# NinV/Background-Debiased-Video-CIL

Measured on AMD Instinct MI355X. Metric: clips/sec fwd+bwd TSM-R50 8x224^2 bs32/GPU, higher is better.
Workload: dtype f32; 1 GPU; TSM-ResNet50 fwd+bwd+SGD step, synthetic 32x8x3x224x224 clips per GPU, 101 classes, SimpleLinear+CrossEntropyLoss, dropout 0.5, random-init weights; fp32 tensors, accumulators and results; conv products: fp32 via 3xbf16 split, 6 MFMA products, fp32 accumulate (dropped terms <= 2^-24 relative); conv_arith=bf16x3, clips_per_gpu=32, global_batch=32, parallelism=dp1

## Files before the change

### background-debiased-video-cil_amd/csrc/conv_mfma.hip

```cpp
#include <stdlib.h>
#include "common.h"

#ifdef BDV_STAMPS
__device__ unsigned long long* g_stamp_buf = nullptr;
__device__ int g_stamp_cap = 0;
#define BDV_STAMP(slot)                                                                                                          \
  do {                                                                                                                           \
    if (threadIdx.x == 0 && g_stamp_buf != nullptr && (int)(blockIdx.x + gridDim.x * blockIdx.y) < g_stamp_cap) {                 \
      unsigned long long* q_ = g_stamp_buf + (size_t)(blockIdx.x + gridDim.x * blockIdx.y) * 8;                                  \
      if ((slot) == 4) asm volatile("s_waitcnt vmcnt(0)" ::: "memory");                                                          \
      q_[slot] = __builtin_amdgcn_s_memtime();                                                                                   \
      if ((slot) == 0) { q_[5] = __builtin_amdgcn_s_memrealtime(); q_[7] = __builtin_amdgcn_s_getreg((4 << 0) | (0 << 6) | (31 << 11)); } \
      if ((slot) == 4) q_[6] = __builtin_amdgcn_s_memrealtime();                                                                 \
    }                                                                                                                            \
  } while (0)
#else
#define BDV_STAMP(slot) do { } while (0)
#endif

namespace {

constexpr int BK = 32;

struct Geom {
  int N, H, W, Cin, Ho, Wo, Cout, R, S, stride, pad, pad_w, T, fold;
  int Rt, st_t;
  float rcp_RS, rcp_S;
  int M;
  int Ktot;
  float rcp_HoWo, rcp_Wo;
  int stagger;
};

typedef unsigned int u32x4 __attribute__((ext_vector_type(4)));
constexpr int kOOB = (int)0x80000000;

__device__ __forceinline__ float4 buf_load16(__amdgpu_buffer_rsrc_t rsrc, int voff, int soff) {
  const u32x4 v = __builtin_amdgcn_raw_buffer_load_b128(rsrc, voff, soff, 0);
  return make_float4(__uint_as_float(v.x), __uint_as_float(v.y), __uint_as_float(v.z), __uint_as_float(v.w));
}

__device__ __forceinline__ void buf_store16(__amdgpu_buffer_rsrc_t rsrc, int voff, float4 v) {
  u32x4 d;
  d.x = __float_as_uint(v.x);
  d.y = __float_as_uint(v.y);
  d.z = __float_as_uint(v.z);
  d.w = __float_as_uint(v.w);
  __builtin_amdgcn_raw_buffer_store_b128(d, rsrc, voff, 0, 0);
}

typedef unsigned int u32x2v __attribute__((ext_vector_type(2)));
template <int ES>
__device__ __forceinline__ float4 buf_ld4(__amdgpu_buffer_rsrc_t rsrc, int voff) {
  if constexpr (ES == 4) {
    return buf_load16(rsrc, voff, 0);
  } else {
    const u32x2v v = __builtin_amdgcn_raw_buffer_load_b64(rsrc, voff, 0, 0);
    return bdv_widen_bf16x4(v.x, v.y);
  }
}
template <int ES>
__device__ __forceinline__ void buf_st4(__amdgpu_buffer_rsrc_t rsrc, int voff, float4 v) {
  if constexpr (ES == 4) {
    buf_store16(rsrc, voff, v);
  } else {
    __builtin_amdgcn_raw_buffer_store_b64((u32x2v){bdv_pack_bf16x2(v.x, v.y), bdv_pack_bf16x2(v.z, v.w)}, rsrc, voff, 0, 0);
  }
}

__device__ __forceinline__ void fast_divmod(int m, int d, float rcp, int& q, int& r) {
  q = (int)((float)m * rcp);
  r = m - q * d;
  if (r < 0) {
    r += d;
    --q;
  }
  if (r >= d) {
    r -= d;
    ++q;
  }
}

template <int LDA, int LDB, int TM, int TN, int MS, int NS, bool SWA, bool SWB>
__device__ __forceinline__ void mma_stage(const float* __restrict__ As, const float* __restrict__ Bs,
                                          f32x16 (&acc)[TM][TN], int wm0, int wn0, int lane) {
  const int r = lane & 31, h = lane >> 5;
  const float* apv[SWA ? 8 : 1];
  const float* bpv[SWB ? 8 : 1];
#pragma unroll
  for (int c = 0; c < (SWA ? 8 : 1); ++c) apv[c] = As + h * LDA + wm0 + (r ^ (4 * c));
#pragma unroll
  for (int c = 0; c < (SWB ? 8 : 1); ++c) bpv[c] = Bs + h * LDB + wn0 + (r ^ (4 * c));
  auto ap = [&](int s, int i) { return apv[SWA ? ((s >> 1) & 7) : 0][2 * s * LDA + MS * i]; };
  auto bp = [&](int s, int j) { return bpv[SWB ? ((s >> 1) & 7) : 0][2 * s * LDB + NS * j]; };
  float a[2][TM], b[2][TN];
#pragma unroll
  for (int i = 0; i < TM; ++i) a[0][i] = ap(0, i);
#pragma unroll
  for (int j = 0; j < TN; ++j) b[0][j] = bp(0, j);
#pragma unroll
  for (int s = 0; s < BK / 2; ++s) {
    const int cur = s & 1, nxt = cur ^ 1;
    if (s + 1 < BK / 2) {
#pragma unroll
      for (int i = 0; i < TM; ++i) a[nxt][i] = ap(s + 1, i);
#pragma unroll
      for (int j = 0; j < TN; ++j) b[nxt][j] = bp(s + 1, j);
    }
#pragma unroll
    for (int i = 0; i < TM; ++i)
#pragma unroll
      for (int j = 0; j < TN; ++j)
        acc[i][j] = __builtin_amdgcn_mfma_f32_32x32x2f32(a[cur][i], b[cur][j], acc[i][j], 0, 0, 0);
    __builtin_amdgcn_sched_group_barrier(0x100, TM + TN, 0);
    __builtin_amdgcn_sched_group_barrier(0x008, TM * TN, 0);
  }
}

__device__ __forceinline__ int shift_class(int c, int fold) {
  return (fold > 0) ? (c < fold ? 1 : (c < 2 * fold ? -1 : 0)) : 0;
}

template <int LD, int PASSES>
__device__ __forceinline__ void store_transposed(float* __restrict__ dst, const float4 (&v)[PASSES], int tid) {
  const int row = tid >> 3, kg = tid & 7;
#pragma unroll
  for (int p = 0; p < PASSES; ++p) {
    float* d = dst + (4 * kg) * LD + ((row + 32 * p) ^ (4 * kg));
    d[0] = v[p].x;
    d[LD] = v[p].y;
    d[2 * LD] = v[p].z;
    d[3 * LD] = v[p].w;
  }
}

template <int LD, int COLS, int PASSES>
__device__ __forceinline__ void store_direct(float* __restrict__ dst, const float4 (&v)[PASSES], int tid) {
  constexpr int V = COLS / 4;
#pragma unroll
  for (int p = 0; p < PASSES; ++p) {
    const int idx = tid + 256 * p;
    const int krow = idx / V, c4 = idx - krow * V;
    *reinterpret_cast<float4*>(dst + krow * LD + 4 * c4) = v[p];
  }
}

__device__ __forceinline__ int acc_row(int reg, int lane) { return (reg & 3) + 8 * (reg >> 2) + 4 * (lane >> 5); }

struct Work {
  int dp_tiles, rem_tiles, split;
};

__device__ __forceinline__ int xcd_remap(int b, int n) {
  const int q = n >> 3, r = n & 7, x = b & 7, j = b >> 3;
  return (x < r ? x * (q + 1) : r * (q + 1) + (x - r) * q) + j;
}

struct WorkItem {
  int tile, kb, ke, pslot;
};

__device__ __forceinline__ WorkItem get_work(int b, const Work& wk, int nk) {
  WorkItem it;
  if (b < wk.dp_tiles) {
    it.tile = xcd_remap(b, wk.dp_tiles);
    it.kb = 0;
    it.ke = nk;
    it.pslot = -1;
  } else {
    const int rem = b - wk.dp_tiles;
    const int rt = rem / wk.split, sl = rem - rt * wk.split;
    it.tile = wk.dp_tiles + rt;
    it.kb = (int)(((long long)sl * nk) / wk.split);
    it.ke = (int)(((long long)(sl + 1) * nk) / wk.split);
    it.pslot = wk.split > 1 ? rem : -1;
  }
  return it;
}

template <int TM, int TN, int NT = 256>
__device__ __forceinline__ void store_partial(float* __restrict__ slab, int pslot, const f32x16 (&acc)[TM][TN], int tid) {
  float* base = slab + (size_t)pslot * (TM * TN * 16) * NT + tid;
#pragma unroll
  for (int i = 0; i < TM; ++i)
#pragma unroll
    for (int j = 0; j < TN; ++j)
#pragma unroll
      for (int e = 0; e < 16; ++e) base[(size_t)((i * TN + j) * 16 + e) * NT] = acc[i][j][e];
}

template <int TM, int TN>
__device__ __forceinline__ void zero_acc(f32x16 (&acc)[TM][TN]) {
#pragma unroll
  for (int i = 0; i < TM; ++i)
#pragma unroll
    for (int j = 0; j < TN; ++j)
#pragma unroll
      for (int e = 0; e < 16; ++e) acc[i][j][e] = 0.f;
}

__device__ __forceinline__ void fprop_store(float* __restrict__ y, const Geom& g, int row, int col, float v) {
  if (row < g.M) y[(size_t)row * g.Cout + col] = v;
}

struct BnStat {
  const void* y;
  const uint32_t* mask;
  const float* mean;
  const float* invstd;
  float* partial;
  int MT;
  const float* rscale;
  const float* rshift;
};

struct StatAcc {
  float4 s1, s2, mu, is;
  __device__ __forceinline__ void init(const BnStat& st, int col) {
    s1 = s2 = make_float4(0.f, 0.f, 0.f, 0.f);
    mu = *reinterpret_cast<const float4*>(st.mean + col);
    is = *reinterpret_cast<const float4*>(st.invstd + col);
  }
  __device__ __forceinline__ static unsigned sign_bits(const BnStat& st, int col, const float4 yv) {
    const float4 rsc = *reinterpret_cast<const float4*>(st.rscale + col), rsh = *reinterpret_cast<const float4*>(st.rshift + col);
    return (fmaf(yv.x, rsc.x, rsh.x) > 0.f ? 1u : 0u) | (fmaf(yv.y, rsc.y, rsh.y) > 0.f ? 2u : 0u) |
           (fmaf(yv.z, rsc.z, rsh.z) > 0.f ? 4u : 0u) | (fmaf(yv.w, rsc.w, rsh.w) > 0.f ? 8u : 0u);
  }
  __device__ __forceinline__ void accumulate(const float4 v, const float4 yv) {
    s1.x += v.x; s1.y += v.y; s1.z += v.z; s1.w += v.w;
    s2.x += v.x * ((yv.x - mu.x) * is.x);
    s2.y += v.y * ((yv.y - mu.y) * is.y);
    s2.z += v.z * ((yv.z - mu.z) * is.z);
    s2.w += v.w * ((yv.w - mu.w) * is.w);
  }
};

template <int BN, int NT = 256>
__device__ __forceinline__ void stat_flush(const StatAcc& a, const BnStat& st, float* __restrict__ smem, int Cin, int mt, int nt,
                                           int tid) {
  constexpr int V = BN / 4, G = NT / V;
  __syncthreads();
  const int grp = tid / V, c4 = tid - grp * V;
  *reinterpret_cast<float4*>(smem + grp * BN + 4 * c4) = a.s1;
  *reinterpret_cast<float4*>(smem + (G + grp) * BN + 4 * c4) = a.s2;
  __syncthreads();
  if (tid < BN) {
    float x = 0.f, y = 0.f;
#pragma unroll
    for (int k = 0; k < G; ++k) {
      x += smem[k * BN + tid];
      y += smem[(G + k) * BN + tid];
    }
    st.partial[(size_t)mt * Cin + nt * BN + tid] = x;
    st.partial[((size_t)st.MT + mt) * Cin + nt * BN + tid] = y;
  }
}

template <int BM, int BN, int WM, int WN, class F>
__device__ __forceinline__ void staged_epilogue(const f32x16 (&acc)[BM / WM / 32][BN / WN / 32], float* __restrict__ smem, int tid,
                                                F&& emit) {
  constexpr int TM = BM / WM / 32, TN = BN / WN / 32;
  constexpr int NT = 64 * WM * WN;
  constexpr int V = BN / 4;
  constexpr int PER = WM * 32 * V / NT;
  const int lane = tid & 63, wave = tid >> 6;
  const int wm = wave / WN, wn0 = (wave % WN) * 32;
#pragma unroll
  for (int i = 0; i < TM; ++i) {
    __syncthreads();
#pragma unroll
    for (int j = 0; j < TN; ++j)
#pragma unroll
      for (int e = 0; e < 16; ++e) smem[(wm * 32 + acc_row(e, lane)) * BN + wn0 + 32 * WN * j + (lane & 31)] = acc[i][j][e];
    __syncthreads();
#pragma unroll
    for (int q = 0; q < PER; ++q) {
      const int idx = tid + NT * q;
      const int lr = idx / V, c4 = idx - lr * V;
      const float4 v = *reinterpret_cast<const float4*>(smem + lr * BN + 4 * c4);
      emit(32 * WM * i + lr, 4 * c4, v);
    }
  }
}


template <int BM, int BN, int WM, int WN, bool DERIVE = true, int ES = 4, bool PIPE = false, class RowMap>
__device__ __forceinline__ void dgrad_epilogue(const f32x16 (&acc)[BM / WM / 32][BN / WN / 32], float* __restrict__ smem, int tid,
                                               void* __restrict__ dx, const void* __restrict__ add_src,
                                               const uint32_t* __restrict__ add_mask, const Geom& g, int mt, int nt, int Mrows,
                                               const BnStat& stat, RowMap&& rowmap) {
  constexpr int TM = BM / WM / 32, TN = BN / WN / 32;
  constexpr int NT = 64 * WM * WN;
  constexpr int V = BN / 4;
  constexpr int PER = WM * 32 * V / NT;
  const int lane = tid & 63, wave = tid >> 6;
  const int wm = wave / WN, wn0 = (wave % WN) * 32;
  const int HW = g.H * g.W;
  const float rcp_HW = 1.0f / (float)HW;
  const int total_bytes = g.N * HW * g.Cin * ES;
  const int mask_bytes = g.N * HW * (g.Cin / 8);
  const __amdgpu_buffer_rsrc_t dxr = __builtin_amdgcn_make_buffer_rsrc((void*)dx, 0, total_bytes, 0x00020000);
  const __amdgpu_buffer_rsrc_t adr =
      __builtin_amdgcn_make_buffer_rsrc((void*)(add_src ? add_src : dx), 0, add_src ? total_bytes : 0, 0x00020000);
  const __amdgpu_buffer_rsrc_t amr =
      __builtin_amdgcn_make_buffer_rsrc((void*)(add_mask ? (const void*)add_mask : (const void*)dx), 0, add_mask ? mask_bytes : 0, 0x00020000);
  const bool do_stat = stat.y != nullptr;
  const __amdgpu_buffer_rsrc_t syr =
      __builtin_amdgcn_make_buffer_rsrc((void*)(do_stat ? stat.y : dx), 0, do_stat ? total_bytes : 0, 0x00020000);
  const __amdgpu_buffer_rsrc_t smr = __builtin_amdgcn_make_buffer_rsrc(
      (void*)(do_stat && stat.mask ? (const void*)stat.mask : (const void*)dx), 0, do_stat && stat.mask ? mask_bytes : 0, 0x00020000);
  const int col = nt * BN + 4 * (tid % V);
  const int cls = shift_class(col, g.fold);
  StatAcc sa;
  if (do_stat) sa.init(stat, col);
  constexpr int HB = PER < 4 ? PER : 4;
  constexpr int NBATCH = PER / HB;
  static_assert(PER % HB == 0, "pieces per pass must be whole batches");
  constexpr int NSETS = PIPE ? 2 : 1;
  float4 a[NSETS][HB], yv[NSETS][HB];
  uint32_t am[NSETS][HB], sm[NSETS][HB];
  int off[NSETS][HB];
  bool zero[NSETS][HB];
  auto issue = [&](int set, int i, int q0) __attribute__((always_inline)) {
#pragma unroll
    for (int u = 0; u < HB; ++u) {
      const int lr = (tid + NT * (q0 + u)) / V;
      const int mrow = mt * BM + 32 * WM * i + lr;
      const bool ok = mrow < Mrows;
      const int row = rowmap(ok ? mrow : 0);
      int drow = row;
      bool z = false;
      if (cls != 0) {
        int n, rem;
        fast_divmod(row, HW, rcp_HW, n, rem);
        const int t = n % g.T;
        const bool inside = (unsigned)(t + cls) < (unsigned)g.T;
        drow = inside ? row + cls * HW : row - cls * (g.T - 1) * HW;
        z = !inside;
      }
      const int o = drow * g.Cin + col;
      off[set][u] = ok ? o * ES : kOOB;
      zero[set][u] = z;
      a[set][u] = buf_ld4<ES>(adr, off[set][u]);
      am[set][u] = add_mask ? __builtin_amdgcn_raw_buffer_load_b32(amr, ok ? (o >> 5) << 2 : kOOB, 0, 0) : 0xffffffffu;
      if (do_stat) {
        yv[set][u] = buf_ld4<ES>(syr, off[set][u]);
        sm[set][u] = stat.mask ? __builtin_amdgcn_raw_buffer_load_b32(smr, ok ? (o >> 5) << 2 : kOOB, 0, 0) : 0xffffffffu;
      }
    }
  };
  auto finish = [&](int set, int q0) __attribute__((always_inline)) {
#pragma unroll
    for (int u = 0; u < HB; ++u) {
      const int lr = (tid + NT * (q0 + u)) / V;
      const float4 t4 = *reinterpret_cast<const float4*>(smem + lr * BN + 4 * (tid % V));
      const int sh = (off[set][u] / ES) & 31;
      const unsigned nib = (am[set][u] >> sh) & 0xFu;
      float4 r = zero[set][u] ? make_float4(0.f, 0.f, 0.f, 0.f) : t4;
      r.x += (nib & 1u) ? a[set][u].x : 0.f;
      r.y += (nib & 2u) ? a[set][u].y : 0.f;
      r.z += (nib & 4u) ? a[set][u].z : 0.f;
      r.w += (nib & 8u) ? a[set][u].w : 0.f;
      buf_st4<ES>(dxr, off[set][u], r);
      if (do_stat && off[set][u] != kOOB) {
        const unsigned sn = (DERIVE && stat.rscale != nullptr) ? StatAcc::sign_bits(stat, col, yv[set][u]) : (sm[set][u] >> sh) & 0xFu;
        float4 gq;
        gq.x = (sn & 1u) ? r.x : 0.f;
        gq.y = (sn & 2u) ? r.y : 0.f;
        gq.z = (sn & 4u) ? r.z : 0.f;
        gq.w = (sn & 8u) ? r.w : 0.f;
        sa.accumulate(gq, yv[set][u]);
      }
    }
  };
  if constexpr (PIPE) issue(0, 0, 0);
#pragma unroll
  for (int i = 0; i < TM; ++i) {
    __syncthreads();
#pragma unroll
    for (int j = 0; j < TN; ++j)
#pragma unroll
      for (int e = 0; e < 16; ++e) smem[(wm * 32 + acc_row(e, lane)) * BN + wn0 + 32 * WN * j + (lane & 31)] = acc[i][j][e];
    __syncthreads();
#pragma unroll
    for (int bq = 0; bq < NBATCH; ++bq) {
      if constexpr (PIPE) {
        const int b = i * NBATCH + bq;
        if (b + 1 < TM * NBATCH) issue((b + 1) & 1, (b + 1) / NBATCH, ((b + 1) % NBATCH) * HB);
        finish(b & 1, bq * HB);
      } else {
        issue(0, i, bq * HB);
        finish(0, bq * HB);
      }
    }
  }
  if (do_stat) stat_flush<BN, NT>(sa, stat, smem, g.Cin, blockIdx.y * (stat.MT >> (gridDim.y == 4 ? 2 : 0)) + mt, nt, tid);
}

template <int BM, int BN, int WM, int WN>
__device__ __forceinline__ void tile_colstats(float* __restrict__ smem, float (&cs)[BN / WN / 32], float (&cq)[BN / WN / 32],
                                              float* __restrict__ bn_partial, int MT, int Cout, int mt, int nt, int tid) {
  constexpr int TN = BN / WN / 32;
  const int lane = tid & 63, wave = tid >> 6;
  const int wm = wave / WN, wn0 = (wave % WN) * 32;
#pragma unroll
  for (int j = 0; j < TN; ++j) {
    cs[j] += __shfl_xor(cs[j], 32, 64);
    cq[j] += __shfl_xor(cq[j], 32, 64);
  }
  __syncthreads();
  if (lane < 32) {
#pragma unroll
    for (int j = 0; j < TN; ++j) {
      smem[wm * BN + wn0 + 32 * WN * j + lane] = cs[j];
      smem[(WM + wm) * BN + wn0 + 32 * WN * j + lane] = cq[j];
    }
  }
  __syncthreads();
  if (tid < BN) {
    float a = 0.f, b = 0.f;
#pragma unroll
    for (int k = 0; k < WM; ++k) {
      a += smem[k * BN + tid];
      b += smem[(WM + k) * BN + tid];
    }
    bn_partial[(size_t)mt * Cout + nt * BN + tid] = a;
    bn_partial[((size_t)MT + mt) * Cout + nt * BN + tid] = b;
  }
}

struct FpropEpi {
  float* bn_partial;
  int MT;
  const float* scale;
  const float* shift;
  const void* res;
  int relu;
  const float* pre_scale;
  const float* pre_shift;
};

template <int BM, int BN, int WM, int WN, int ES = 4>
__device__ __forceinline__ void fprop_affine_epilogue(const f32x16 (&acc)[BM / WM / 32][BN / WN / 32], float* __restrict__ smem,
                                                      void* __restrict__ y, const Geom& g, const FpropEpi& epi, int mt, int nt,
                                                      int tid) {
  constexpr int TM = BM / WM / 32, TN = BN / WN / 32;
  constexpr int NT = 64 * WM * WN;
  constexpr int V = BN / 4;
  constexpr int PER = WM * 32 * V / NT;
  constexpr int HB = PER < 4 ? PER : 4;
  const int lane = tid & 63, wave = tid >> 6;
  const int wm = wave / WN, wn0 = (wave % WN) * 32;
  const int total_bytes = g.M * g.Cout * ES;
  const __amdgpu_buffer_rsrc_t yr = __builtin_amdgcn_make_buffer_rsrc((void*)y, 0, total_bytes, 0x00020000);
  const __amdgpu_buffer_rsrc_t rr =
      __builtin_amdgcn_make_buffer_rsrc((void*)(epi.res ? epi.res : (const void*)y), 0, epi.res ? total_bytes : 0, 0x00020000);
  const int col = nt * BN + 4 * (tid % V);
  const float4 sc = *reinterpret_cast<const float4*>(epi.scale + col);
  const float4 sh = *reinterpret_cast<const float4*>(epi.shift + col);
#pragma unroll
  for (int i = 0; i < TM; ++i) {
    __syncthreads();
#pragma unroll
    for (int j = 0; j < TN; ++j)
#pragma unroll
      for (int e = 0; e < 16; ++e) smem[(wm * 32 + acc_row(e, lane)) * BN + wn0 + 32 * WN * j + (lane & 31)] = acc[i][j][e];
    __syncthreads();
#pragma unroll
    for (int q0 = 0; q0 < PER; q0 += HB) {
      float4 v[HB], r[HB];
      int off[HB];
#pragma unroll
      for (int u = 0; u < HB; ++u) {
        const int lr = (tid + NT * (q0 + u)) / V;
        const int row = mt * BM + 32 * WM * i + lr;
        off[u] = row < g.M ? (row * g.Cout + col) * ES : kOOB;
        v[u] = *reinterpret_cast<const float4*>(smem + lr * BN + 4 * (tid % V));
        r[u] = buf_ld4<ES>(rr, off[u]);
      }
#pragma unroll
      for (int u = 0; u < HB; ++u) {
        float4 o;
        o.x = v[u].x * sc.x + sh.x + r[u].x;
        o.y = v[u].y * sc.y + sh.y + r[u].y;
        o.z = v[u].z * sc.z + sh.z + r[u].z;
        o.w = v[u].w * sc.w + sh.w + r[u].w;
        if (epi.relu) {
          o.x = fmaxf(o.x, 0.f);
          o.y = fmaxf(o.y, 0.f);
          o.z = fmaxf(o.z, 0.f);
          o.w = fmaxf(o.w, 0.f);
        }
        buf_st4<ES>(yr, off[u], o);
      }
    }
  }
}

template <int BM, int BN, int WM, int WN, int ES = 4>
__device__ __forceinline__ void fprop_epilogue(const f32x16 (&acc)[BM / WM / 32][BN / WN / 32], float* __restrict__ smem,
                                               void* __restrict__ y, const Geom& g, const FpropEpi& epi, int mt, int nt, int tid) {
  constexpr int TM = BM / WM / 32, TN = BN / WN / 32;
  const int lane = tid & 63, wave = tid >> 6;
  const int wm0 = (wave / WN) * 32;
  if (epi.scale != nullptr) {
    fprop_affine_epilogue<BM, BN, WM, WN, ES>(acc, smem, y, g, epi, mt, nt, tid);
    return;
  }
  float* const bn_partial = epi.bn_partial;
  const int MT = epi.MT;
  staged_epilogue<BM, BN, WM, WN>(acc, smem, tid, [&](int tr, int tc, float4 v) {
    const int row = mt * BM + tr;
    if (row < g.M) act_st4<ES>(y, ((size_t)row * g.Cout + nt * BN + tc) >> 2, v);
  });
  if (bn_partial != nullptr) {
    float cs[TN], cq[TN];
#pragma unroll
    for (int j = 0; j < TN; ++j) cs[j] = cq[j] = 0.f;
#pragma unroll
    for (int i = 0; i < TM; ++i)
#pragma unroll
      for (int j = 0; j < TN; ++j)
#pragma unroll
        for (int e = 0; e < 16; ++e) {
          const int row = mt * BM + wm0 + 32 * WM * i + acc_row(e, lane);
          const float v = row < g.M ? acc[i][j][e] : 0.f;
          cs[j] += v;
          cq[j] += v * v;
        }
    tile_colstats<BM, BN, WM, WN>(smem, cs, cq, bn_partial, MT, g.Cout, mt, nt, tid);
  }
}

template <int BM, int BN, int WM, int WN>
__global__ __launch_bounds__(256, 3) void conv_fprop_kernel(const float* __restrict__ x, const float* __restrict__ w,
                                                          float* __restrict__ y, Geom g, int NT, Work wk,
                                                          float* __restrict__ slab, FpropEpi epi) {
  constexpr int LDA = BM, LDB = BN;
  constexpr int TM = BM / WM / 32, TN = BN / WN / 32;
  constexpr int AP = BM / 32, BP = BN / 32;
  __shared__ __attribute__((aligned(16))) float smem[BK * (LDA + LDB)];
  float* const As = smem;
  float* const Bs = smem + BK * LDA;

  const int nk = g.Ktot / BK;
  const WorkItem it = get_work(blockIdx.x, wk, nk);
  const int mt = it.tile / NT, nt = it.tile - mt * NT;

  const int tid = threadIdx.x;
// ... 465 lines not shown
#pragma unroll
    for (int i = 0; i < TM; ++i)
#pragma unroll
      for (int j = 0; j < TN; ++j)
#pragma unroll
        for (int e = 0; e < 16; ++e) acc[i][j][e] += src[(size_t)((i * TN + j) * 16 + e) * NTHR];
  }
  fprop_epilogue<BM, BN, WM, WN>(acc, smem, y, g, epi, mt, nt, tid);
}

template <int BM, int BN, int WM, int WN>
__global__ __launch_bounds__(256, 3) void conv_dgrad_kernel(const float* __restrict__ dy, const float* __restrict__ w,
                                                          float* __restrict__ dx, const float* __restrict__ add_src,
                                                          const uint32_t* __restrict__ add_mask, Geom g, int NT, Work wk,
                                                          float* __restrict__ slab, BnStat stat) {
  constexpr int LDA = BM, LDB = BN;
  constexpr int TM = BM / WM / 32, TN = BN / WN / 32;
  constexpr int AP = BM / 32, BP = BN / 32;
  constexpr int BV = BN / 4;
  constexpr int AOFF = (BK * LDA + 3) & ~3;
  constexpr int SMEM = (AOFF + BK * LDB) > (WM * 32 * BN) ? (AOFF + BK * LDB) : (WM * 32 * BN);
  __shared__ __attribute__((aligned(16))) float smem[SMEM];
  float* const As = smem;
  float* const Bs = smem + AOFF;

  const int st = g.stride;
  const int ph = blockIdx.y / st, pw = blockIdx.y - ph * st;
  const int Hc = (g.H - ph + st - 1) / st, Wc = (g.W - pw + st - 1) / st;
  const int Mc = g.N * Hc * Wc;
  const int MT = (Mc + BM - 1) / BM;
  const int r0 = (ph + g.pad) % st, s0 = (pw + g.pad_w) % st;
  const int nr = r0 < g.R ? (g.R - r0 + st - 1) / st : 0;
  const int ns = s0 < g.S ? (g.S - s0 + st - 1) / st : 0;
  const int bh = (ph + g.pad - r0) / st, bw = (pw + g.pad_w - s0) / st;
  const int ntap = nr * ns;
  const int nk = ntap * g.Cout / BK;

  int mt, nt;
  WorkItem it;
  if (st == 1) {
    it = get_work(blockIdx.x, wk, nk);
    mt = it.tile / NT;
    nt = it.tile - mt * NT;
  } else {
    const int id = blockIdx.x;
    const int xcd = id & 7, jj = id >> 3;
    mt = (jj / NT) * 8 + xcd;
    nt = jj % NT;
    if (mt >= MT) return;
    it.tile = 0;
    it.kb = 0;
    it.ke = nk;
    it.pslot = -1;
  }

  const int tid = threadIdx.x;
  const int lane = tid & 63, wave = tid >> 6;
  const int wm0 = (wave / WN) * 32, wn0 = (wave % WN) * 32;
  const int arow = tid >> 3, kg = tid & 7;
  const int HcWc = Hc * Wc;
  const int RS = g.R * g.S;
  const __amdgpu_buffer_rsrc_t yr = __builtin_amdgcn_make_buffer_rsrc((void*)dy, 0, g.N * g.Ho * g.Wo * g.Cout * 4, 0x00020000);
  const __amdgpu_buffer_rsrc_t wr = __builtin_amdgcn_make_buffer_rsrc((void*)w, 0, g.Cout * RS * g.Cin * 4, 0x00020000);

  int a_base[AP], a_h[AP], a_w[AP];
#pragma unroll
  for (int p = 0; p < AP; ++p) {
    const int m = mt * BM + arow + 32 * p;
    const bool ok = m < Mc;
    const int mm = ok ? m : 0;
    const int n = mm / HcWc;
    const int rem = mm - n * HcWc;
    const int hc = rem / Wc, wc = rem - hc * Wc;
    a_h[p] = ok ? hc + bh : -(1 << 20);
    a_w[p] = wc + bw;
    a_base[p] = ((n * g.Ho + hc + bh) * g.Wo + wc + bw) * g.Cout * 4 + 16 * kg;
  }
  int b_base[BP];
#pragma unroll
  for (int p = 0; p < BP; ++p) {
    const int idx = tid + 256 * p;
    const int krow = idx / BV, c4 = idx - krow * BV;
    b_base[p] = (krow * RS * g.Cin + nt * BN + 4 * c4) * 4;
  }

  int chunk = ntap > 0 ? it.kb / ntap : 0, ir, is;
  {
    const int ct = ntap > 0 ? it.kb - chunk * ntap : 0;
    ir = ns > 0 ? ct / ns : 0;
    is = ct - ir * ns;
  }

  float4 ra[AP], rb[BP];
  auto load = [&]() {
    const int tap = (r0 + ir * st) * g.S + (s0 + is * st);
    const int koff_a = (chunk * BK - (ir * g.Wo + is) * g.Cout) * 4;
    const int koff_b = (chunk * BK * RS + tap) * g.Cin * 4;
#pragma unroll
    for (int p = 0; p < AP; ++p) {
      const bool v = (unsigned)(a_h[p] - ir) < (unsigned)g.Ho && (unsigned)(a_w[p] - is) < (unsigned)g.Wo;
      ra[p] = buf_load16(yr, (a_base[p] + koff_a) | (v ? 0 : kOOB), 0);
    }
#pragma unroll
    for (int p = 0; p < BP; ++p) rb[p] = buf_load16(wr, b_base[p], koff_b);
    is += 1;
    const int w1 = (is == ns) ? 1 : 0;
    is = w1 ? 0 : is;
    ir += w1;
    const int w2 = (ir == nr) ? 1 : 0;
    ir = w2 ? 0 : ir;
    chunk += w2;
  };

  f32x16 acc[TM][TN];
  zero_acc<TM, TN>(acc);

  if (it.ke > it.kb) {
    load();
    for (int kt = it.kb; kt < it.ke; ++kt) {
      __syncthreads();
      store_transposed<LDA, AP>(As, ra, tid);
      store_direct<LDB, BN, BP>(Bs, rb, tid);
      __syncthreads();
      if (kt + 1 < it.ke) load();
      mma_stage<LDA, LDB, TM, TN, 32 * WM, 32 * WN, true, false>(As, Bs, acc, wm0, wn0, lane);
    }
  }
  if (it.pslot >= 0) {
    store_partial<TM, TN>(slab, it.pslot, acc, tid);
    return;
  }

  dgrad_epilogue<BM, BN, WM, WN, BN == 64>(acc, smem, tid, dx, add_src, add_mask, g, mt, nt, Mc, stat, [&](int mrow) {
    if (st == 1) return mrow;
    const int n = mrow / HcWc;
    const int rem = mrow - n * HcWc;
    const int hc = rem / Wc;
    return (n * g.H + hc * st + ph) * g.W + (rem - hc * Wc) * st + pw;
  });
}

template <int BM, int BN, int WM, int WN, bool BPRE = false>
__global__ __launch_bounds__(256, 2) void conv_dgrad_x3_kernel(const float* __restrict__ dy, const float* __restrict__ wt,
                                                          float* __restrict__ dx, const float* __restrict__ add_src,
                                                          const uint32_t* __restrict__ add_mask, Geom g, int NT, Work wk,
                                                          float* __restrict__ slab, BnStat stat) {
  constexpr int TM = BM / WM / 32, TN = BN / WN / 32;
  constexpr int AP = BM / 32, BP = BN / 32;
  static_assert(3 * (BM + BN) * X3_LDK * 2 >= WM * 32 * BN * 4, "the epilogue stages a tile pass in the same LDS");
  __shared__ __attribute__((aligned(16))) unsigned short smem16[3 * (BM + BN) * X3_LDK];
  unsigned short* const As = smem16;
  unsigned short* const Bs = smem16 + 3 * BM * X3_LDK;
  float* const smem = reinterpret_cast<float*>(smem16);

  const int st = g.stride;
  const int ph = blockIdx.y / st, pw = blockIdx.y - ph * st;
  const int Hc = (g.H - ph + st - 1) / st, Wc = (g.W - pw + st - 1) / st;
  const int Mc = g.N * Hc * Wc;
  const int MT = (Mc + BM - 1) / BM;
  const int r0 = (ph + g.pad) % st, s0 = (pw + g.pad_w) % st;
  const int nr = r0 < g.R ? (g.R - r0 + st - 1) / st : 0;
  const int ns = s0 < g.S ? (g.S - s0 + st - 1) / st : 0;
  const int bh = (ph + g.pad - r0) / st, bw = (pw + g.pad_w - s0) / st;
  const int ntap = nr * ns;
  const int nk = ntap * g.Cout / BK;

  int mt, nt;
  WorkItem it;
  if (st == 1) {
    it = get_work(blockIdx.x, wk, nk);
    mt = it.tile / NT;
    nt = it.tile - mt * NT;
  } else {
    const int id = blockIdx.x;
    const int xcd = id & 7, jj = id >> 3;
    mt = (jj / NT) * 8 + xcd;
    nt = jj % NT;
    if (mt >= MT) return;
    it.tile = 0;
    it.kb = 0;
    it.ke = nk;
    it.pslot = -1;
  }

  const int tid = threadIdx.x;
  const int lane = tid & 63, wave = tid >> 6;
  const int wm0 = (wave / WN) * 32, wn0 = (wave % WN) * 32;
  const int arow = tid >> 3, kg = tid & 7;
  const int HcWc = Hc * Wc;
  const int RS = g.R * g.S;
  const __amdgpu_buffer_rsrc_t yr = __builtin_amdgcn_make_buffer_rsrc((void*)dy, 0, g.N * g.Ho * g.Wo * g.Cout * 4, 0x00020000);
  const __amdgpu_buffer_rsrc_t wr = __builtin_amdgcn_make_buffer_rsrc((void*)wt, 0, BPRE ? 3 * g.Cout * RS * g.Cin * 2 : g.Cout * RS * g.Cin * 4, 0x00020000);
  constexpr int BQ = BN * 4 / 256;
  const int brow = tid >> 2, bc = tid & 3;
  const int plane_bytes = g.Cout * RS * g.Cin * 2;
  const int nchunk = g.Cout / BK;

  int a_base[AP], a_h[AP], a_w[AP];
#pragma unroll
  for (int p = 0; p < AP; ++p) {
    const int m = mt * BM + arow + 32 * p;
    const bool ok = m < Mc;
    const int mm = ok ? m : 0;
    const int n = mm / HcWc;
    const int rem = mm - n * HcWc;
    const int hc = rem / Wc, wc = rem - hc * Wc;
    a_h[p] = ok ? hc + bh : -(1 << 20);
    a_w[p] = wc + bw;
    a_base[p] = ((n * g.Ho + hc + bh) * g.Wo + wc + bw) * g.Cout * 4 + 16 * kg;
  }
  int b_base[BP];
#pragma unroll
  for (int p = 0; p < BP; ++p) b_base[p] = ((nt * BN + arow + 32 * p) * g.Cout + 4 * kg) * 4;

  int chunk = ntap > 0 ? it.kb / ntap : 0, ir, is;
  {
    const int ct = ntap > 0 ? it.kb - chunk * ntap : 0;
    ir = ns > 0 ? ct / ns : 0;
    is = ct - ir * ns;
  }

  float4 ra[AP], rb[BP];
  u32x4 rbp[BPRE ? 3 * BQ : 1];
  auto load = [&]() {
    const int tap = (r0 + ir * st) * g.S + (s0 + is * st);
    const int koff_a = (chunk * BK - (ir * g.Wo + is) * g.Cout) * 4;
    const int koff_b = (tap * g.Cin * g.Cout + chunk * BK) * 4;
#pragma unroll
    for (int p = 0; p < AP; ++p) {
      const bool v = (unsigned)(a_h[p] - ir) < (unsigned)g.Ho && (unsigned)(a_w[p] - is) < (unsigned)g.Wo;
      ra[p] = buf_load16(yr, (a_base[p] + koff_a) | (v ? 0 : kOOB), 0);
    }
    if (BPRE) {
#pragma unroll
      for (int pl = 0; pl < 3; ++pl)
#pragma unroll
        for (int q = 0; q < BQ; ++q)
          rbp[pl * BQ + q] = __builtin_amdgcn_raw_buffer_load_b128(wr, (nt * BN + brow + 64 * q) * 64 + 16 * bc + pl * plane_bytes,
                                                                   (tap * nchunk + chunk) * g.Cin * 64, 0);
    } else {
#pragma unroll
      for (int p = 0; p < BP; ++p) rb[p] = buf_load16(wr, b_base[p], koff_b);
    }
    is += 1;
    const int w1 = (is == ns) ? 1 : 0;
    is = w1 ? 0 : is;
    ir += w1;
    const int w2 = (ir == nr) ? 1 : 0;
    ir = w2 ? 0 : ir;
    chunk += w2;
  };

  f32x16 acc[TM][TN];
  zero_acc<TM, TN>(acc);

  if (it.ke > it.kb) {
    load();
    for (int kt = it.kb; kt < it.ke; ++kt) {
      __syncthreads();
      store_split3<BM, AP>(As, ra, tid);
      if (BPRE) {
#pragma unroll
        for (int pl = 0; pl < 3; ++pl)
#pragma unroll
          for (int q = 0; q < BQ; ++q) *reinterpret_cast<u32x4*>(Bs + (pl * BN + brow + 64 * q) * X3_LDK + 8 * bc) = rbp[pl * BQ + q];
      } else {
        store_split3<BN, BP>(Bs, rb, tid);
      }
      __syncthreads();
      if (kt + 1 < it.ke) load();
      mma_stage_x3<TM, TN, 32 * WM, 32 * WN, BM, BN>(As, Bs, acc, wm0, wn0, lane);
    }
  }
  if (it.pslot >= 0) {
    store_partial<TM, TN>(slab, it.pslot, acc, tid);
    return;
  }

  dgrad_epilogue<BM, BN, WM, WN, true, 4, true>(acc, smem, tid, dx, add_src, add_mask, g, mt, nt, Mc, stat, [&](int mrow) {
    if (st == 1) return mrow;
    const int n = mrow / HcWc;
    const int rem = mrow - n * HcWc;
    const int hc = rem / Wc;
    return (n * g.H + hc * st + ph) * g.W + (rem - hc * Wc) * st + pw;
  });
}

template <int BM, int BN, int WM, int WN>
__global__ __launch_bounds__(64 * WM * WN) void conv_dgrad_fixup_kernel(const float* __restrict__ slab, float* __restrict__ dx,
                                                                const float* __restrict__ add_src,
                                                                const uint32_t* __restrict__ add_mask, Geom g, int NT, Work wk,
                                                                BnStat stat) {
  constexpr int TM = BM / WM / 32, TN = BN / WN / 32;
  constexpr int NACC = TM * TN * 16;
  constexpr int NTHR = 64 * WM * WN;
  __shared__ __attribute__((aligned(16))) float smem[WM * 32 * BN];
  const int rt = blockIdx.x, tile = wk.dp_tiles + rt;
  const int mt = tile / NT, nt = tile - mt * NT;
  const int tid = threadIdx.x;
  f32x16 acc[TM][TN];
  zero_acc<TM, TN>(acc);
  for (int sl = 0; sl < wk.split; ++sl) {
    const float* src = slab + (size_t)(rt * wk.split + sl) * NACC * NTHR + tid;
#pragma unroll
    for (int i = 0; i < TM; ++i)
#pragma unroll
      for (int j = 0; j < TN; ++j)
#pragma unroll
        for (int e = 0; e < 16; ++e) acc[i][j][e] += src[(size_t)((i * TN + j) * 16 + e) * NTHR];
  }
  dgrad_epilogue<BM, BN, WM, WN>(acc, smem, tid, dx, add_src, add_mask, g, mt, nt, g.M, stat, [](int mrow) { return mrow; });
}

template <int BM, int BN, int WM, int WN, bool C4, bool INCR>
__global__ __launch_bounds__(256, 3) void conv_wgrad_kernel(const float* __restrict__ dy, const float* __restrict__ x,
                                                          float* __restrict__ slab, Geom g, int MTw, int NTw,
                                                          int kt_per_split) {
  constexpr int LDA = BM, LDB = BN;
  constexpr int TM = BM / WM / 32, TN = BN / WN / 32;
  constexpr int AP = BM / 32, BP = BN / 32;
  constexpr int AV = BM / 4, BV = BN / 4;
  __shared__ __attribute__((aligned(16))) float smem[BK * (LDA + LDB)];
  float* const As = smem;
  float* const Bs = smem + BK * LDA;

  const int tiles = MTw * NTw;
  const int wi = xcd_remap(blockIdx.x, gridDim.x);
  const int split = wi / tiles;
  const int tile = wi - split * tiles;
  const int mt = tile % MTw, nt = tile / MTw;
  const int tid = threadIdx.x;
  const int lane = tid & 63, wave = tid >> 6;
  const int wm0 = (wave / WN) * 32, wn0 = (wave % WN) * 32;
  const int HoWo = g.Ho * g.Wo;
  const int frame_bytes = g.H * g.W * g.Cin * 4;
  const __amdgpu_buffer_rsrc_t xr = __builtin_amdgcn_make_buffer_rsrc((void*)x, 0, g.N * frame_bytes, 0x00020000);
  const __amdgpu_buffer_rsrc_t yr = __builtin_amdgcn_make_buffer_rsrc((void*)dy, 0, g.M * g.Cout * 4, 0x00020000);

  int a_off[AP];
#pragma unroll
  for (int p = 0; p < AP; ++p) {
    const int idx = tid + 256 * p;
    const int krow = idx / AV, c4 = idx - krow * AV;
    a_off[p] = (krow * g.Cout + mt * BM + 4 * c4) * 4;
  }
  int b_krow[BP], b_off[BP], b_r[BP], b_s[BP], b_cls[BP];
  bool b_cok[BP];
#pragma unroll
  for (int p = 0; p < BP; ++p) {
    const int idx = tid + 256 * p;
    const int krow = idx / BV, c4 = idx - krow * BV;
    b_krow[p] = krow;
    int tap, ci;
    if (C4) {
      const int ncol = nt * BN + 4 * c4;
      tap = ncol / g.Cin;
      ci = ncol - tap * g.Cin;
      b_cok[p] = ncol < g.Ktot;
    } else {
      const int per_tap = g.Cin / BN;
      tap = nt / per_tap;
      ci = (nt - tap * per_tap) * BN + 4 * c4;
      b_cok[p] = true;
    }
    b_r[p] = tap / g.S - g.pad;
    b_s[p] = tap % g.S - g.pad_w;
    b_cls[p] = shift_class(ci, g.fold);
    b_off[p] = ((b_r[p] * g.W + b_s[p]) * g.Cin + ci) * 4 + b_cls[p] * frame_bytes;
  }

  const int kt_begin = split * kt_per_split;
  const int nkt_all = (g.M + BK - 1) / BK;
  const int kt_end = min(kt_begin + kt_per_split, nkt_all);

  const int st = g.stride;
  const int d_ho = BK / g.Wo, d_wo = BK - d_ho * g.Wo;
  const int wrap_w = g.Wo * st, wrap_h = g.Ho * st;
  const int px = g.Cin * 4;
  const int inc0 = (d_ho * st * g.W + d_wo * st) * px;
  const int inc1 = (st * g.W - wrap_w) * px;
  const int inc2 = (g.H * g.W - wrap_h * g.W) * px;
  int s_hi[BP], s_wi[BP], s_t[BP], s_off[BP];
  if (INCR) {
#pragma unroll
    for (int p = 0; p < BP; ++p) {
      const int m = split * kt_per_split * BK + b_krow[p];
      const int n = m / HoWo;
      const int rem = m - n * HoWo;
      const int ho = rem / g.Wo, wo = rem - ho * g.Wo;
      s_hi[p] = ho * st;
      s_wi[p] = wo * st;
      s_t[p] = n % g.T;
      s_off[p] = ((n * g.H + s_hi[p]) * g.W + s_wi[p]) * px + b_off[p];
    }
  }

  float4 ra[AP], rb[BP];
  auto load = [&](int kt) {
    const int m0 = kt * BK;
#pragma unroll
    for (int p = 0; p < AP; ++p)
      ra[p] = buf_load16(yr, a_off[p] + m0 * g.Cout * 4, 0);
#pragma unroll
    for (int p = 0; p < BP; ++p) {
      const int m = m0 + b_krow[p];
      const bool mok = m < g.M;
      int hi, wi, t, off;
      if (INCR) {
        hi = s_hi[p];
        wi = s_wi[p];
        t = s_t[p];
        off = s_off[p];
        const int w2 = wi + d_wo * st;
        const bool c1 = w2 >= wrap_w;
        s_wi[p] = c1 ? w2 - wrap_w : w2;
        const int h2 = hi + d_ho * st + (c1 ? st : 0);
        const bool c2 = h2 >= wrap_h;
        s_hi[p] = c2 ? h2 - wrap_h : h2;
        const int t2 = t + (c2 ? 1 : 0);
        s_t[p] = t2 == g.T ? 0 : t2;
        s_off[p] = off + inc0 + (c1 ? inc1 : 0) + (c2 ? inc2 : 0);
      } else {
        const int mm = mok ? m : 0;
        const int n = mm / HoWo;
        const int rem = mm - n * HoWo;
        const int ho = rem / g.Wo;
        hi = ho * st;
        wi = (rem - ho * g.Wo) * st;
        t = n % g.T;
        off = ((n * g.H + hi) * g.W + wi) * px + b_off[p];
      }
      const bool v = mok && b_cok[p] && (unsigned)(hi + b_r[p]) < (unsigned)g.H && (unsigned)(wi + b_s[p]) < (unsigned)g.W &&
                     (unsigned)(t + b_cls[p]) < (unsigned)g.T;
      rb[p] = buf_load16(xr, off | (v ? 0 : kOOB), 0);
    }
  };

  f32x16 acc[TM][TN];
// ... 2022 lines not shown
```

Baseline: 612.0 clips/s.

## Prefetch dgrad epilogue residual loads before the K loop via stateful epilogue object

Turns the dgrad epilogue into a struct so the kernel can build it before the main K loop and issue the first batch of residual, mask and BN-stat loads ahead of the MFMA loop. The epilogue then runs two sets deep, overlapping the global-load latency of the epilogue with the mainloop compute. It also replaces the modulo by T with a reciprocal-based fast_divmod and adds optional timing stamps. The trade-off is higher register pressure from keeping the prefetched values live across the K loop, which could lower occupancy.

```diff
diff --git a/background-debiased-video-cil_amd/csrc/conv_mfma.hip b/background-debiased-video-cil_amd/csrc/conv_mfma.hip
--- a/background-debiased-video-cil_amd/csrc/conv_mfma.hip
+++ b/background-debiased-video-cil_amd/csrc/conv_mfma.hip
@@ -2,20 +2,29 @@
 #include "common.h"
 
 #ifdef BDV_STAMPS
+#define BDV_STAMP_WORDS 32
 __device__ unsigned long long* g_stamp_buf = nullptr;
 __device__ int g_stamp_cap = 0;
 #define BDV_STAMP(slot)                                                                                                          \
   do {                                                                                                                           \
     if (threadIdx.x == 0 && g_stamp_buf != nullptr && (int)(blockIdx.x + gridDim.x * blockIdx.y) < g_stamp_cap) {                 \
-      unsigned long long* q_ = g_stamp_buf + (size_t)(blockIdx.x + gridDim.x * blockIdx.y) * 8;                                  \
+      unsigned long long* q_ = g_stamp_buf + (size_t)(blockIdx.x + gridDim.x * blockIdx.y) * BDV_STAMP_WORDS;                    \
       if ((slot) == 4) asm volatile("s_waitcnt vmcnt(0)" ::: "memory");                                                          \
       q_[slot] = __builtin_amdgcn_s_memtime();                                                                                   \
       if ((slot) == 0) { q_[5] = __builtin_amdgcn_s_memrealtime(); q_[7] = __builtin_amdgcn_s_getreg((4 << 0) | (0 << 6) | (31 << 11)); } \
       if ((slot) == 4) q_[6] = __builtin_amdgcn_s_memrealtime();                                                                 \
     }                                                                                                                            \
   } while (0)
+#define BDV_STAMP_EPI_VAL(k, v)                                                                                                  \
+  do {                                                                                                                           \
+    if (threadIdx.x == 0 && g_stamp_buf != nullptr && (int)(blockIdx.x + gridDim.x * blockIdx.y) < g_stamp_cap)                   \
+      g_stamp_buf[(size_t)(blockIdx.x + gridDim.x * blockIdx.y) * BDV_STAMP_WORDS + 8 + (k)] = (v);                              \
+  } while (0)
+#define BDV_STAMP_EPI(k) BDV_STAMP_EPI_VAL(k, __builtin_amdgcn_s_memtime())
 #else
 #define BDV_STAMP(slot) do { } while (0)
+#define BDV_STAMP_EPI(k) do { } while (0)
+#define BDV_STAMP_EPI_VAL(k, v) do { } while (0)
 #endif
 
 namespace {
@@ -284,44 +293,55 @@
 }
 
 
-template <int BM, int BN, int WM, int WN, bool DERIVE = true, int ES = 4, bool PIPE = false, class RowMap>
-__device__ __forceinline__ void dgrad_epilogue(const f32x16 (&acc)[BM / WM / 32][BN / WN / 32], float* __restrict__ smem, int tid,
-                                               void* __restrict__ dx, const void* __restrict__ add_src,
-                                               const uint32_t* __restrict__ add_mask, const Geom& g, int mt, int nt, int Mrows,
-                                               const BnStat& stat, RowMap&& rowmap) {
-  constexpr int TM = BM / WM / 32, TN = BN / WN / 32;
-  constexpr int NT = 64 * WM * WN;
-  constexpr int V = BN / 4;
-  constexpr int PER = WM * 32 * V / NT;
-  const int lane = tid & 63, wave = tid >> 6;
-  const int wm = wave / WN, wn0 = (wave % WN) * 32;
-  const int HW = g.H * g.W;
-  const float rcp_HW = 1.0f / (float)HW;
-  const int total_bytes = g.N * HW * g.Cin * ES;
-  const int mask_bytes = g.N * HW * (g.Cin / 8);
-  const __amdgpu_buffer_rsrc_t dxr = __builtin_amdgcn_make_buffer_rsrc((void*)dx, 0, total_bytes, 0x00020000);
-  const __amdgpu_buffer_rsrc_t adr =
-      __builtin_amdgcn_make_buffer_rsrc((void*)(add_src ? add_src : dx), 0, add_src ? total_bytes : 0, 0x00020000);
-  const __amdgpu_buffer_rsrc_t amr =
-      __builtin_amdgcn_make_buffer_rsrc((void*)(add_mask ? (const void*)add_mask : (const void*)dx), 0, add_mask ? mask_bytes : 0, 0x00020000);
-  const bool do_stat = stat.y != nullptr;
-  const __amdgpu_buffer_rsrc_t syr =
-      __builtin_amdgcn_make_buffer_rsrc((void*)(do_stat ? stat.y : dx), 0, do_stat ? total_bytes : 0, 0x00020000);
-  const __amdgpu_buffer_rsrc_t smr = __builtin_amdgcn_make_buffer_rsrc(
-      (void*)(do_stat && stat.mask ? (const void*)stat.mask : (const void*)dx), 0, do_stat && stat.mask ? mask_bytes : 0, 0x00020000);
-  const int col = nt * BN + 4 * (tid % V);
-  const int cls = shift_class(col, g.fold);
+template <int BM, int BN, int WM, int WN, bool DERIVE, int ES, int PIPE, class RowMap>
+struct DgradEpi {
+  static constexpr int TM = BM / WM / 32, TN = BN / WN / 32;
+  static constexpr int NT = 64 * WM * WN;
+  static constexpr int V = BN / 4;
+  static constexpr int PER = WM * 32 * V / NT;
+  static constexpr int HB = PER < 4 ? PER : 4;
+  static constexpr int NBATCH = PER / HB;
+  static_assert(PER % HB == 0, "pieces per pass must be whole batches");
+  static constexpr int AHEAD = PIPE;
+  static constexpr int NSETS = AHEAD + 1;
+
+  const Geom& g;
+  const BnStat& stat;
+  RowMap rowmap;
+  const uint32_t* add_mask;
+  int tid, mt, nt, Mrows, HW, col, cls;
+  float rcp_HW, rcp_T;
+  bool do_stat;
+  __amdgpu_buffer_rsrc_t dxr, adr, amr, syr, smr;
   StatAcc sa;
-  if (do_stat) sa.init(stat, col);
-  constexpr int HB = PER < 4 ? PER : 4;
-  constexpr int NBATCH = PER / HB;
-  static_assert(PER % HB == 0, "pieces per pass must be whole batches");
-  constexpr int NSETS = PIPE ? 2 : 1;
   float4 a[NSETS][HB], yv[NSETS][HB];
   uint32_t am[NSETS][HB], sm[NSETS][HB];
   int off[NSETS][HB];
   bool zero[NSETS][HB];
-  auto issue = [&](int set, int i, int q0) __attribute__((always_inline)) {
+
+  __device__ __forceinline__ DgradEpi(int tid_, void* __restrict__ dx, const void* __restrict__ add_src,
+                                      const uint32_t* __restrict__ add_mask_, const Geom& g_, int mt_, int nt_, int Mrows_,
+                                      const BnStat& stat_, RowMap rowmap_)
+      : g(g_), stat(stat_), rowmap(rowmap_), add_mask(add_mask_), tid(tid_), mt(mt_), nt(nt_), Mrows(Mrows_) {
+    HW = g.H * g.W;
+    rcp_HW = 1.0f / (float)HW;
+    rcp_T = 1.0f / (float)g.T;
+    const int total_bytes = g.N * HW * g.Cin * ES;
+    const int mask_bytes = g.N * HW * (g.Cin / 8);
+    dxr = __builtin_amdgcn_make_buffer_rsrc((void*)dx, 0, total_bytes, 0x00020000);
+    adr = __builtin_amdgcn_make_buffer_rsrc((void*)(add_src ? add_src : dx), 0, add_src ? total_bytes : 0, 0x00020000);
+    amr = __builtin_amdgcn_make_buffer_rsrc((void*)(add_mask ? (const void*)add_mask : (const void*)dx), 0, add_mask ? mask_bytes : 0,
+                                            0x00020000);
+    do_stat = stat.y != nullptr;
+    syr = __builtin_amdgcn_make_buffer_rsrc((void*)(do_stat ? stat.y : dx), 0, do_stat ? total_bytes : 0, 0x00020000);
+    smr = __builtin_amdgcn_make_buffer_rsrc((void*)(do_stat && stat.mask ? (const void*)stat.mask : (const void*)dx), 0,
+                                            do_stat && stat.mask ? mask_bytes : 0, 0x00020000);
+    col = nt * BN + 4 * (tid % V);
+    cls = shift_class(col, g.fold);
+    if (do_stat) sa.init(stat, col);
+  }
+
+  __device__ __forceinline__ void issue(int set, int i, int q0) {
 #pragma unroll
     for (int u = 0; u < HB; ++u) {
       const int lr = (tid + NT * (q0 + u)) / V;
@@ -331,9 +351,9 @@
       int drow = row;
       bool z = false;
       if (cls != 0) {
-        int n, rem;
+        int n, rem, clip, t;
         fast_divmod(row, HW, rcp_HW, n, rem);
-        const int t = n % g.T;
+        fast_divmod(n, g.T, rcp_T, clip, t);
         const bool inside = (unsigned)(t + cls) < (unsigned)g.T;
         drow = inside ? row + cls * HW : row - cls * (g.T - 1) * HW;
         z = !inside;
@@ -348,8 +368,9 @@
         sm[set][u] = stat.mask ? __builtin_amdgcn_raw_buffer_load_b32(smr, ok ? (o >> 5) << 2 : kOOB, 0, 0) : 0xffffffffu;
       }
     }
-  };
-  auto finish = [&](int set, int q0) __attribute__((always_inline)) {
+  }
+
+  __device__ __forceinline__ void finish(int set, int q0, const float* __restrict__ smem) {
 #pragma unroll
     for (int u = 0; u < HB; ++u) {
       const int lr = (tid + NT * (q0 + u)) / V;
@@ -372,29 +393,52 @@
         sa.accumulate(gq, yv[set][u]);
       }
     }
-  };
-  if constexpr (PIPE) issue(0, 0, 0);
-#pragma unroll
-  for (int i = 0; i < TM; ++i) {
-    __syncthreads();
-#pragma unroll
-    for (int j = 0; j < TN; ++j)
-#pragma unroll
-      for (int e = 0; e < 16; ++e) smem[(wm * 32 + acc_row(e, lane)) * BN + wn0 + 32 * WN * j + (lane & 31)] = acc[i][j][e];
-    __syncthreads();
-#pragma unroll
-    for (int bq = 0; bq < NBATCH; ++bq) {
-      if constexpr (PIPE) {
-        const int b = i * NBATCH + bq;
-        if (b + 1 < TM * NBATCH) issue((b + 1) & 1, (b + 1) / NBATCH, ((b + 1) % NBATCH) * HB);
-        finish(b & 1, bq * HB);
-      } else {
-        issue(0, i, bq * HB);
-        finish(0, bq * HB);
+  }
+
+  __device__ __forceinline__ void prime() { issue(0, 0, 0); }
+
+  __device__ __forceinline__ void run(const f32x16 (&acc)[TM][TN], float* __restrict__ smem) {
+    const int lane = tid & 63, wave = tid >> 6;
+    const int wm = wave / WN, wn0 = (wave % WN) * 32;
+    if constexpr (PIPE == 1) issue(0, 0, 0);
+    if constexpr (PIPE == 2 && TM * NBATCH > 1) issue(1, 1 / NBATCH, (1 % NBATCH) * HB);
+#pragma unroll
+    for (int i = 0; i < TM; ++i) {
+      __syncthreads();
+#pragma unroll
+      for (int j = 0; j < TN; ++j)
+#pragma unroll
+        for (int e = 0; e < 16; ++e) smem[(wm * 32 + acc_row(e, lane)) * BN + wn0 + 32 * WN * j + (lane & 31)] = acc[i][j][e];
+      __syncthreads();
+      BDV_STAMP_EPI(i * (NBATCH + 1));
+#pragma unroll
+      for (int bq = 0; bq < NBATCH; ++bq) {
+        if constexpr (PIPE != 0) {
+          const int b = i * NBATCH + bq, nb = b + AHEAD;
+          if (nb < TM * NBATCH) issue(nb % NSETS, nb / NBATCH, (nb % NBATCH) * HB);
+          finish(b % NSETS, bq * HB, smem);
+        } else {
+          issue(0, i, bq * HB);
+          finish(0, bq * HB, smem);
+        }
+        BDV_STAMP_EPI(i * (NBATCH + 1) + 1 + bq);
       }
     }
-  }
-  if (do_stat) stat_flush<BN, NT>(sa, stat, smem, g.Cin, blockIdx.y * (stat.MT >> (gridDim.y == 4 ? 2 : 0)) + mt, nt, tid);
+    BDV_STAMP_EPI_VAL(21, nt * BN < 2 * g.fold ? 1 : 0);
+    BDV_STAMP_EPI(22);
+    if (do_stat) stat_flush<BN, NT>(sa, stat, smem, g.Cin, blockIdx.y * (stat.MT >> (gridDim.y == 4 ? 2 : 0)) + mt, nt, tid);
+    BDV_STAMP_EPI(23);
+  }
+};
+
+template <int BM, int BN, int WM, int WN, bool DERIVE = true, int ES = 4, int PIPE = 0, class RowMap>
+__device__ __forceinline__ void dgrad_epilogue(const f32x16 (&acc)[BM / WM / 32][BN / WN / 32], float* __restrict__ smem, int tid,
+                                               void* __restrict__ dx, const void* __restrict__ add_src,
+                                               const uint32_t* __restrict__ add_mask, const Geom& g, int mt, int nt, int Mrows,
+                                               const BnStat& stat, RowMap&& rowmap) {
+  static_assert(PIPE != 2, "PIPE = 2: the kernel owns the DgradEpi and primes it before its K loop");
+  DgradEpi<BM, BN, WM, WN, DERIVE, ES, PIPE, RowMap> epi(tid, dx, add_src, add_mask, g, mt, nt, Mrows, stat, rowmap);
+  epi.run(acc, smem);
 }
 
 template <int BM, int BN, int WM, int WN>
@@ -1166,6 +1210,7 @@
   unsigned short* const As = smem16;
   unsigned short* const Bs = smem16 + 3 * BM * X3_LDK;
   float* const smem = reinterpret_cast<float*>(smem16);
+  BDV_STAMP(0);
 
   const int st = g.stride;
   const int ph = blockIdx.y / st, pw = blockIdx.y - ph * st;
@@ -1268,36 +1313,41 @@
   f32x16 acc[TM][TN];
   zero_acc<TM, TN>(acc);
 
-  if (it.ke > it.kb) {
-    load();
-    for (int kt = it.kb; kt < it.ke; ++kt) {
-      __syncthreads();
-      store_split3<BM, AP>(As, ra, tid);
-      if (BPRE) {
-#pragma unroll
-        for (int pl = 0; pl < 3; ++pl)
-#pragma unroll
-          for (int q = 0; q < BQ; ++q) *reinterpret_cast<u32x4*>(Bs + (pl * BN + brow + 64 * q) * X3_LDK + 8 * bc) = rbp[pl * BQ + q];
-      } else {
-        store_split3<BN, BP>(Bs, rb, tid);
-      }
-      __syncthreads();
-      if (kt + 1 < it.ke) load();
-      mma_stage_x3<TM, TN, 32 * WM, 32 * WN, BM, BN>(As, Bs, acc, wm0, wn0, lane);
-    }
-  }
-  if (it.pslot >= 0) {
-    store_partial<TM, TN>(slab, it.pslot, acc, tid);
-    return;
-  }
-
-  dgrad_epilogue<BM, BN, WM, WN, true, 4, true>(acc, smem, tid, dx, add_src, add_mask, g, mt, nt, Mc, stat, [&](int mrow) {
+  auto rowmap = [&](int mrow) {
     if (st == 1) return mrow;
     const int n = mrow / HcWc;
     const int rem = mrow - n * HcWc;
     const int hc = rem / Wc;
     return (n * g.H + hc * st + ph) * g.W + (rem - hc * Wc) * st + pw;
-  });
+  };
+  DgradEpi<BM, BN, WM, WN, true, 4, 2, decltype(rowmap)> epi(tid, dx, add_src, add_mask, g, mt, nt, Mc, stat, rowmap);
+
+  if (it.ke > it.kb) load();
+  if (it.pslot < 0) epi.prime();
+  for (int kt = it.kb; kt < it.ke; ++kt) {
+    __syncthreads();
+    store_split3<BM, AP>(As, ra, tid);
+    if (BPRE) {
+#pragma unroll
+      for (int pl = 0; pl < 3; ++pl)
+#pragma unroll
+        for (int q = 0; q < BQ; ++q) *reinterpret_cast<u32x4*>(Bs + (pl * BN + brow + 64 * q) * X3_LDK + 8 * bc) = rbp[pl * BQ + q];
+    } else {
+      store_split3<BN, BP>(Bs, rb, tid);
+    }
+    __syncthreads();
+    if (kt == it.kb) BDV_STAMP(1);
+    if (kt + 1 < it.ke) load();
+    mma_stage_x3<TM, TN, 32 * WM, 32 * WN, BM, BN>(As, Bs, acc, wm0, wn0, lane);
+  }
+  BDV_STAMP(2);
+  if (it.pslot >= 0) {
+    store_partial<TM, TN>(slab, it.pslot, acc, tid);
+    return;
+  }
+  epi.run(acc, smem);
+  BDV_STAMP(3);
+  BDV_STAMP(4);
 }
 
 template <int BM, int BN, int WM, int WN>
```

Result: no change. 611.6 clips/s, median of 5 (-0.1%).
